# aiortc/aioquic

Hardware: AMD Instinct MI355X
Metric: GiB/s device-resident AEAD protect+unprotect, 1200B packets, 1/2/4/8 MI355X (higher is better)
Workload: dtype u8

## Files before the change

aioquic_amd/csrc/qpp_device.h:

```cpp
#pragma once

#include <hip/hip_runtime.h>
#include <stdint.h>

#include "../../include/quic_pp.h"

namespace qpp {


struct AesTables {
    uint8_t sbox[256];
    uint32_t te0[256];
};

constexpr uint8_t gf8_mul(uint8_t a, uint8_t b)
{
    uint8_t r = 0;
    for (int i = 0; i < 8; ++i) {
        if (b & 1) r ^= a;
        a = (uint8_t)((a << 1) ^ ((a & 0x80) ? 0x1b : 0));
        b >>= 1;
    }
    return r;
}
// ... 396 lines not shown
        uint32_t e[2][16];
        lds_phase_prio(true);
#pragma unroll
        for (int b = 0; b < 2; ++b) {
#pragma unroll
            for (int col = 0; col < 4; ++col) {
                e[b][4 * col + 0] = T.t0(s[b][col]);
                e[b][4 * col + 1] = T.t1(s[b][(col + 1) & 3]);
                e[b][4 * col + 2] = T.t2r(s[b][(col + 2) & 3]);
                e[b][4 * col + 3] = T.t3r(s[b][(col + 3) & 3]);
            }
        }
        __builtin_amdgcn_sched_barrier(0);
        lds_phase_prio(false);
#pragma unroll
        for (int b = 0; b < 2; ++b) {
#pragma unroll
            for (int col = 0; col < 4; ++col)
                s[b][col] = xor3(e[b][4 * col], e[b][4 * col + 1],
                                 rotl(xor3(e[b][4 * col + 2], e[b][4 * col + 3], k[col]), 16));
        }
    }
    const uint32_t *k = rk + 4 * NR;
    uint32_t f[2][16];
    lds_phase_prio(true);
#pragma unroll
    for (int b = 0; b < 2; ++b) {
#pragma unroll
        for (int col = 0; col < 4; ++col) {
            f[b][4 * col + 0] = T.fr0(s[b][col]);
            f[b][4 * col + 1] = T.fr1(s[b][(col + 1) & 3]);
            f[b][4 * col + 2] = T.fr2(s[b][(col + 2) & 3]);
            f[b][4 * col + 3] = T.fr3(s[b][(col + 3) & 3]);
        }
    }
    __builtin_amdgcn_sched_barrier(0);
    lds_phase_prio(false);
    uint32_t o[2][4];
#pragma unroll
    for (int b = 0; b < 2; ++b) {
#pragma unroll
        for (int col = 0; col < 4; ++col)
            o[b][col] = fin_col(f[b][4 * col], f[b][4 * col + 1], f[b][4 * col + 2], f[b][4 * col + 3], k[col]);
    }
    o0 = u32x4{o[0][0], o[0][1], o[0][2], o[0][3]};
    o1 = u32x4{o[1][0], o[1][1], o[1][2], o[1][3]};
}


__device__ __forceinline__ u32x4 ghash_mul(u32x4 x, const uint8_t *lds, uint32_t tab)
{
    u32x4 acc = {0, 0, 0, 0};
    uint32_t xw[4] = {x.x, x.y, x.z, x.w};
#pragma unroll
    for (int d = 0; d < 4; ++d) {
        uint32_t hi = xw[d] & 0xF0F0F0F0u;
        uint32_t lo = (xw[d] << 4) & 0xF0F0F0F0u;
#pragma unroll
        for (int b = 0; b < 4; ++b) {
            const int wlo = 2 * (4 * d + b), whi = wlo + 1;
            const uint32_t sel = 0x0c0c0c00u | (uint32_t)b;
            uint32_t alo = __builtin_amdgcn_perm(0u, lo, sel);
            uint32_t ahi = __builtin_amdgcn_perm(0u, hi, sel);
            u32x4 e0 = *(const u32x4 *)(lds + tab + wlo * 256 + alo);
            u32x4 e1 = *(const u32x4 *)(lds + tab + whi * 256 + ahi);
            acc = xor3(acc, e0, e1);
        }
    }
    return acc;
}

template <int W0, int W1>
struct Gh5Grp {
    u32x2 lo[W1 - W0], hi[W1 - W0];
    __device__ __forceinline__ void issue(const uint32_t (&xw)[4], const uint8_t *base, uint32_t tsel)
    {
#pragma unroll
        for (int i = 0; i < W1 - W0; ++i) {
            const int w = W0 + i, sb = 5 * w, d = sb >> 5, off = sb & 31;
            uint32_t e;
            if (off <= 27) asm("v_bfe_u32 %0, %1, %2, 5" : "=v"(e) : "v"(xw[d]), "i"(off));
            else if (d < 3) e = __builtin_amdgcn_alignbit(xw[d + 1], xw[d], off) & 31u;
            else e = xw[3] >> off;
            const uint32_t a = (e << 3) | tsel;
            lo[i] = *(const u32x2 *)(base + w * 256 + a);
            hi[i] = *(const u32x2 *)(base + kGh5Hi + w * 256 + a);
        }
    }
    __device__ __forceinline__ void consume(u32x4 &acc) const
    {
        constexpr int n = W1 - W0;
#pragma unroll
        for (int i = 0; i + 1 < n; i += 2) {
            acc.x = xor3(acc.x, lo[i].x, lo[i + 1].x);
            acc.y = xor3(acc.y, lo[i].y, lo[i + 1].y);
            acc.z = xor3(acc.z, hi[i].x, hi[i + 1].x);
            acc.w = xor3(acc.w, hi[i].y, hi[i + 1].y);
        }
        if constexpr (n & 1) {
            acc.x ^= lo[n - 1].x;
            acc.y ^= lo[n - 1].y;
            acc.z ^= hi[n - 1].x;
            acc.w ^= hi[n - 1].y;
        }
    }
};

__device__ __forceinline__ u32x4 ghash_mul_lds5(u32x4 x, const uint8_t *base, uint32_t tsel)
{
    const uint32_t xw[4] = {x.x, x.y, x.z, x.w};
// ... 84 lines not shown
```

aioquic_amd/csrc/qpp_engine.hip:

```cpp
#include <hip/hip_runtime.h>

#include "qpp_chacha.h"
#include "qpp_gf128.h"
#include "qpp_device.h"
#include "qpp_hkdf.h"
#include "qpp_internal.h"

namespace qpp {

__constant__ AesTables c_aes = kAesTables;

constexpr int kSetupWG = 256;
constexpr int kScratch = 112;
constexpr int kScrEj0 = 48, kScrPark = 64, kScrHdr = 96;
constexpr uint32_t kNoSlot = 0xffffffffu;
constexpr uint32_t kFlagReject = 0x8000u;
constexpr int kChachaWpe = 4;

constexpr int kChRegion = 64 * 16 + 16;
constexpr int kChStage = 4 * kChRegion;

#ifndef QPP_CH_POLY4
#define QPP_CH_POLY4 1
#endif
// ... 336 lines not shown
#define QPP_PROBE_AT(i) probe_mark(i)
#define QPP_PROBE_COUNT()                                                                     \
    do {                                                                                      \
        const uint32_t w_ = blockIdx.x * (blockDim.x / 64) + (threadIdx.x >> 6);              \
        if (w_ < kProbeWaves && __lane_id() == __ffsll((long long)__ballot(1)) - 1)           \
            atomicAdd(&g_probe[(size_t)w_ * kProbeSlots + kProbeItems], 1ull);                \
    } while (0)
#else
#define QPP_PROBE_COUNT() ((void)0)
#define QPP_PROBE_AT(i) ((void)0)
#endif

__device__ __forceinline__ void park(const Pkt &P, uint8_t *scr, bool mask = true)
{
    if (mask) *(u32x4 *)(scr + kScrPark) = P.mask;
    *(u32x4 *)(scr + kScrPark + 16) =
        u32x4{(uint32_t)P.pn, (uint32_t)(P.pn >> 32),
              P.fbm | (uint32_t)P.pn_off << 8 | (uint32_t)P.pn_len << 24 | (uint32_t)P.hp << 28,
              (uint32_t)P.hlen | (uint32_t)P.clen << 16};
}
__device__ __forceinline__ Pkt unpark(const uint8_t *scr, const uint8_t *src, uint8_t *dst, bool mask = true)
{
    Pkt P;
    const u32x4 w = *(const u32x4 *)(scr + kScrPark + 16);
    P.src = src;
    P.dst = dst;
    P.hlen = (int)(w.w & 0xffff);
    P.clen = (int)(w.w >> 16);
    P.mask = mask ? *(const u32x4 *)(scr + kScrPark) : zero4();
    P.pn = (uint64_t)w.y << 32 | w.x;
    P.fbm = w.z & 0xff;
    P.pn_off = (int)((w.z >> 8) & 0xffff);
    P.pn_len = (int)((w.z >> 24) & 0xf);
    P.hp = (w.z >> 28) & 1;
    P.status = QPP_S_OK;
    P.nonce = u32x4{0, 0, 0, 0};
    return P;
}

__device__ __forceinline__ uint32_t lds_ld(const uint32_t *p)
{
    return __hip_atomic_load(p, __ATOMIC_RELAXED, __HIP_MEMORY_SCOPE_WORKGROUP);
}
__device__ __forceinline__ void lds_st(uint32_t *p, uint32_t v)
{
    __hip_atomic_store(p, v, __ATOMIC_RELAXED, __HIP_MEMORY_SCOPE_WORKGROUP);
}

struct GhashTabs {
    const uint8_t *lds;
    const uint8_t *gtab;
    const uint32_t *wslot;
    const uint32_t *went;
    __device__ __forceinline__ uint32_t t4() const
    {
        return __builtin_amdgcn_readfirstlane(lds_ld(went)) * (uint32_t)kGhLdsEntry;
    }
    __device__ __forceinline__ const uint8_t *global(uint32_t pw) const
    {
        const uint32_t s = __builtin_amdgcn_readfirstlane(lds_ld(wslot));
        return gtab + (size_t)s * kGhashTabBytes + pw * (uint32_t)kGhashPowBytes;
    }
};

template <int BPL>
__device__ __forceinline__ int gcm_pad(int n_g)
{
    constexpr int QS = 4 * BPL;
    return QS * ((n_g + QS - 1) / QS) - n_g;
}

template <int BPL>
__device__ __forceinline__ bool gcm_fast_hp(int hlen, int clen)
{
    if constexpr (BPL != 2) {
        return false;
    } else {
        const int n_a = (hlen + 15) >> 4, n_c = (clen + 15) >> 4, za = n_a > 0 ? 1 : 0;
        return gcm_pad<BPL>(za + n_c + 1) + za <= 6 && clen >= 19;
    }
}

__device__ __forceinline__ void buf_st_part(__amdgpu_buffer_rsrc_t r, uint32_t off, u32x4 v, int n)
{
    const int nd = n >> 2, rb = n & 3;
    if (nd > 0) __builtin_amdgcn_raw_buffer_store_b32(v.x, r, (int)off, 0, 0);
    if (nd > 1) __builtin_amdgcn_raw_buffer_store_b32(v.y, r, (int)off + 4, 0, 0);
    if (nd > 2) __builtin_amdgcn_raw_buffer_store_b32(v.z, r, (int)off + 8, 0, 0);
    if (rb) {
        uint32_t t = nd == 0 ? v.x : nd == 1 ? v.y : nd == 2 ? v.z : v.w;
        const int o = (int)off + 4 * nd;
        if (rb & 2) {
            __builtin_amdgcn_raw_buffer_store_b16((unsigned short)t, r, o, 0, 0);
            t >>= 16;
        }
        if (rb & 1) __builtin_amdgcn_raw_buffer_store_b8((unsigned char)t, r, o + (rb & 2), 0, 0);
    }
}

__device__ __forceinline__ void write_header_v(const Pkt &P, int sub, bool masked, int rlen, u32x4 h0,
                                               bool have_h0)
{
    const int n_a = (P.hlen + 15) >> 4;
    for (int q = sub; q < n_a; q += 4) {
        const int nb = min(16, P.hlen - 16 * q);
        u32x4 h = (q == 0 && have_h0) ? h0 : ld_win(P.src + 16 * q, nb, P.src, P.src + rlen);
        if (masked) h ^= hp_pattern(16 * q, P.mask, P.fbm, P.pn_off, P.pn_len);
        st_part(P.dst + 16 * q, h, nb);
    }
}

template <int NR, bool ENC, int BPL, int SUITE, bool PRIO>
__device__ __forceinline__ u32x4 gcm_packet(const Pkt &P, const KeySlot *ks, const u32x4 h0,
                                            const uint32_t *rk, int sub, const GhashTabs &G,
                                            const uint8_t *te, const Bufs &B, uint32_t ioff, uint32_t ooff,
                                            u32x4 &got_tag, uint32_t pbase = 0u)
{
    const LdsTe T{te, (lane_fresh() & 31) * 4};
    const int hlen = P.hlen, clen = P.clen;
    const int n_a = (hlen + 15) >> 4, n_c = (clen + 15) >> 4, za = n_a > 0 ? 1 : 0;
    const int n_g = za + n_c + 1, pad = gcm_pad<BPL>(n_g), S = (n_g + pad) / (4 * BPL);
    const int rlen = hlen + clen + (ENC ? 0 : QPP_TAG_LEN);
    const bool tiny = rlen < 16;
    const uint32_t t4 = G.t4();
    const u32x4 tiny_in = tiny ? ld_part(P.src, rlen) : zero4();
    const int q = pad + za;
    const uint32_t cin = ioff + (uint32_t)hlen, cout = ooff + (uint32_t)hlen;
    auto ct_load = [&](int i) -> uint32_t {
        if (i < 0 || 16 * i >= clen) return kOob;
        return cin + (uint32_t)(ENC ? min(16 * i, clen - 16) : 16 * i);
    };
    u32x4 nxt0 = {0, 0, 0, 0}, nxt1 = {0, 0, 0, 0};
    if constexpr (BPL == 2) {
        nxt0 = __builtin_amdgcn_raw_buffer_load_b128(B.in, (int)ct_load(sub - q), 0, 0);
        nxt1 = __builtin_amdgcn_raw_buffer_load_b128(B.in, (int)ct_load(sub - q + 4), 0, 0);
    }

    u32x4 z = {0, 0, 0, 0};
    for (int g = 0; g < n_a; ++g) {
        u32x4 a;
        if (tiny) {
            a = tiny_in;
        } else if (g == 0) {
            a = h0;
        } else {
            const int ld = min(16 * g, rlen - 16);
            a = shr_bytes(__builtin_amdgcn_raw_buffer_load_b128(B.in, (int)(ioff + ld), 0, 0),
                          16 * g - ld);
        }
        a = keep_bytes(a, min(16, hlen - 16 * g));
        if (!ENC && P.hp) a ^= hp_pattern(16 * g, P.mask, P.fbm, P.pn_off, P.pn_len);
        if (g > 0) z = ghash_mul_global(z, G.global(0));
        z ^= a;
    }
    if (!ENC || !P.hp) write_header_v(P, sub, !ENC && P.hp, rlen, tiny ? tiny_in : h0, true);
    const bool fast_hp = ENC && P.hp && gcm_fast_hp<BPL>(hlen, clen);
    u32x4 acc = (BPL == 1 && za && sub == pad) ? z : u32x4{0, 0, 0, 0};
    const CtrCache cc = ctr_cache(P.nonce, rk, T);
    const uint32_t lens_h = bswap((uint32_t)hlen * 8u);

    auto close = [&](u32x4 ksl) {
        const uint32_t lf = lane_fresh();
        acc = ghash_mul_global(acc, G.global(3u - (lf & 3)));
        if ((lf & 3) == 3) acc ^= ksl;
    };
    auto blk_out = [&](int i, u32x4 ksb, u32x4 raw) -> u32x4 {
        const bool is_ct = i >= 0 && 16 * i < clen;
        u32x4 x = {0, 0, 0, 0}, out = {0, 0, 0, 0};
        uint32_t soff = kOob;
        if (is_ct) {
            const int nb = clen - 16 * i;
            if (__builtin_expect(nb >= 16, 1)) {
                out = raw ^ ksb;
                x = ENC ? out : raw;
                soff = cout + 16u * (uint32_t)i;
            } else {
                const u32x4 cur = ENC ? shr_bytes(raw, 16 - nb) : raw;
                out = cur ^ ksb;
                x = keep_bytes(ENC ? out : cur, nb);
                buf_st_part(B.out, cout + 16u * (uint32_t)i, out, nb);
            }
        } else if (i >= 0 && 16 * i < clen + 16) {
            x = u32x4{0u, lens_h, 0u, bswap((uint32_t)clen * 8u)};
        }
        __builtin_amdgcn_raw_buffer_store_b128(out, B.out, (int)soff, 0, 0);
        return x;
    };
    auto step = [&](int i, bool last, auto first_c, u32x4 raw) {
        (void)first_c;
        const LdsTe Tl{te, (lane_fresh() & 31) * 4};
        const bool is_ct = i >= 0 && 16 * i < clen;
        const u32x4 ksb = aes_ctr<NR>(cc, is_ct ? (uint32_t)(i + 2) : 1u, rk, Tl);
        acc ^= blk_out(i, ksb, raw);
        __builtin_amdgcn_sched_barrier(0);
        if (!last) acc = ghash_mul_h4(acc, G.lds, t4);
        else close(ksb);
    };
    auto step2 = [&](int i, bool last, u32x4 raw0, u32x4 raw1, auto first_c) {
        constexpr bool first = decltype(first_c)::value;
        const LdsTe Tl{te, (lane_fresh() & 31) * 4};
        const uint32_t cb0 = (i >= 0 && 16 * i < clen) ? (uint32_t)(i + 2) : 1u;
        const uint32_t cb1 = (i + 4 >= 0 && 16 * (i + 4) < clen) ? (uint32_t)(i + 6) : 1u;
        u32x4 ks0, ks1;
        if (first && pad >= 4) {
            ks0 = zero4();
            ks1 = aes_ctr<NR>(cc, cb1, rk, Tl);
        } else {
            aes_ctr2<NR>(cc, cb0, cb1, rk, Tl, ks0, ks1);
        }
        u32x4 x0 = blk_out(i, ks0, raw0);
        u32x4 x1 = blk_out(i + 4, ks1, raw1);
        if constexpr (first) {
            if constexpr (ENC) {
                if (fast_hp) {
                    u32x4 c0 = (i == 0) ? x0 : (i + 4 == 0) ? x1 : zero4();
                    u32x4 c1 = (i == 1) ? x0 : (i + 4 == 1) ? x1 : zero4();
// ... 432 lines not shown
        uint8_t *dst = P.dst;
        P = unpark(scr, src, dst, !ENC);
    }
    const int L = chunks & 3;
    const int nb = chunks > 0 ? n_c - 4 * (chunks - 1) : 1;
    const int role = (sub - L - 1) & 3;
    auto power = [&](int e) -> P130 {
        P130 x;
#pragma unroll
        for (int l = 0; l < 5; ++l) x.v[l] = pw[5 * e + l];
        return x;
    };
    const u32x4 lens = u32x4{(uint32_t)P.hlen, 0u, (uint32_t)P.clen, 0u};
    const P130 lb = p130_block(lens);
    P130 a = acc;
#pragma unroll
    for (int l = 0; l < 5; ++l) a.v[l] += role == 3 ? lb.v[l] : 0u;
    const P130 m = p130_mul(a, power(role == 0 ? kPw8 : role == 1 ? kPw1 + 3 : role == 2 ? kPwOne : kPw1));
    P130 u = m, v = p130_zero();
#pragma unroll
    for (int l = 0; l < 5; ++l) {
        u.v[l] = role == 3 ? 0u : m.v[l];
        v.v[l] = role == 3 ? m.v[l] : 0u;
    }
    const P130 sum = p130_add(p130_mul(p130_quad_sum(u), power(kPw1 + nb)), p130_quad_sum(v));
    const u32x4 sw = *(const u32x4 *)(scr + kScrEj0);
    const u32x4 tag = p130_finish(sum, sw.x, sw.y, sw.z, sw.w);
    if (ENC) {
        if (sub == 0) st16(pout + P.clen, tag);
        if (P.hp) protect_finish_hp<QPP_CHACHA20_POLY1305>(P, ks, sub, scr, tag, ConstTe{}, h0);
    } else {
        const u32x4 got = ld16(pin + P.clen);
        const u32x4 diff = got ^ tag;
        if ((diff.x | diff.y | diff.z | diff.w) != 0) {
            P.status = QPP_S_DECRYPT;
            wipe_payload(P, sub, [&](int i) { return ((i >> 2) + 1) & 3; });
        }
    }
    QPP_PROBE_AT(7);
}

template <bool ENC>
__device__ __forceinline__ void write_result(qpp_result *res, uint32_t p, int sub, const Pkt &P)
{
    if (sub != 0) return;
    const uint32_t out_len =
        P.status == QPP_S_OK ? (uint32_t)(P.hlen + P.clen + (ENC ? QPP_TAG_LEN : 0)) : 0u;
    res[p] = qpp_result{P.pn, (uint16_t)P.status, (uint16_t)P.hlen, out_len};
}



constexpr int kTabEntries = 4;
template <int WG>
constexpr int gcm_tab_entries() { return WG == 512 ? 1 : kTabEntries; }
static_assert(kGhLdsEntry % 1024 == 0, "LDS-DMA pieces of 1 KiB");

__device__ uint32_t g_qpp_watchdog;

__device__ uint32_t g_qpp_spin_tab = 1u << 22;
__device__ uint32_t g_qpp_spin_lone = 1u << 18;
__device__ uint32_t g_qpp_pair_delay = 0u;

template <int WG, int NE = gcm_tab_entries<WG>()>
struct __attribute__((aligned(16))) GcmSmem {
    uint8_t h4[NE][kGhLdsEntry];
    uint8_t te[kTeBytes];
    uint32_t eslot[NE];
    uint32_t eref[NE];
    uint32_t eready[NE];
    uint32_t eused[NE];

    uint32_t lock, tick, next;
    uint32_t exited;
    uint32_t wslot[WG / 64];
    uint32_t went[WG / 64];
};

template <int WG>
__device__ uint32_t tab_acquire(GcmSmem<WG> &sm, const uint8_t *gtab, uint32_t cur)
{
    const uint32_t spin = __builtin_nontemporal_load(&g_qpp_spin_tab);
    typedef const __attribute__((address_space(1))) void *gptr_t;
    typedef __attribute__((address_space(3))) void *lptr_t;
    uint32_t e = kNoSlot, load = 0;
#pragma unroll 1
    for (uint32_t it = 0; it < spin; ++it) {
        uint32_t got = kNoSlot, ld = 0;
        if (lane_fresh() == 0) {
            while (atomicCAS(&sm.lock, 0u, 1u) != 0u) __builtin_amdgcn_s_sleep(1);
            int hit = -1, vic = -1;
            uint32_t best = 0xffffffffu;
#pragma unroll
            for (int i = 0; i < gcm_tab_entries<WG>(); ++i) {
                const uint32_t s = lds_ld(&sm.eslot[i]);
                const uint32_t r = lds_ld(&sm.eref[i]);
                const uint32_t u = lds_ld(&sm.eused[i]);
                if (s == cur) hit = i;
                else if (r == 0u && u < best) {
                    best = u;
                    vic = i;
                }
            }
            if (hit < 0 && vic >= 0) {
                hit = vic;
                ld = 1;
                lds_st(&sm.eslot[vic], cur);
                lds_st(&sm.eready[vic], 0u);
            }
            if (hit >= 0) {
                got = (uint32_t)hit;
                atomicAdd(&sm.eref[hit], 1u);
                const uint32_t t = lds_ld(&sm.tick) + 1u;
                lds_st(&sm.tick, t);
                lds_st(&sm.eused[hit], t);
            }
            asm volatile("s_waitcnt lgkmcnt(0)" ::: "memory");
            atomicExch(&sm.lock, 0u);
        }
        got = __builtin_amdgcn_readfirstlane(got);
        if (got != kNoSlot) {
            e = got;
            load = __builtin_amdgcn_readfirstlane(ld);
            break;
        }
        __builtin_amdgcn_s_sleep(8);
    }
    if (e == kNoSlot) return e;
    if (load) {
        const uint8_t *src = gtab + (size_t)cur * kGhashTabBytes + kGh5Off;
        const uint32_t l = lane_fresh();
#pragma unroll
        for (int c = 0; c < kGhLdsEntry / 1024; ++c)
            __builtin_amdgcn_global_load_lds((gptr_t)(src + c * 1024 + l * 16), (lptr_t)(sm.h4[e] + c * 1024),
                                             16, 0, 0);
        asm volatile("s_waitcnt vmcnt(0)" ::: "memory");
        if (lane_fresh() == 0) lds_st(&sm.eready[e], 1u);
    } else {
        bool ready = false;
#pragma unroll 1
        for (uint32_t it = 0; it < spin; ++it) {
            if (__builtin_amdgcn_readfirstlane(lds_ld(&sm.eready[e]))) {
                ready = true;
                break;
            }
            __builtin_amdgcn_s_sleep(2);
        }
        if (!ready) {
            if (lane_fresh() == 0) atomicSub(&sm.eref[e], 1u);
            return kNoSlot;
        }
    }
    return e;
}

template <int WG>
__device__ __forceinline__ void tab_release(GcmSmem<WG> &sm, uint32_t e)
{
    if (lane_fresh() == 0) atomicSub(&sm.eref[e], 1u);
}

#ifdef QPP_STUDY_SYNTH
__device__ __forceinline__ qpp_desc study_desc(const qpp_desc *, uint32_t p)
{
    return qpp_desc{1200ull * p, 1200ull * p, 1173u, 11, 0, (uint64_t)p, 0u, p};
}
#define QPP_DESC(i) study_desc(desc, (i))
#else
#define QPP_DESC(i) desc[i]
#endif

#ifndef QPP_POOL_DIV
#define QPP_POOL_DIV 12
#endif
constexpr uint32_t kPoolDiv = QPP_POOL_DIV;
#ifndef QPP_POOL512
#define QPP_POOL512 0
#endif
#ifndef QPP_COMBO_PRIO
#define QPP_COMBO_PRIO 0
#endif
#ifndef QPP_SHARE_PRIO
#define QPP_SHARE_PRIO 0
#endif
#ifndef QPP_PRIO512
#define QPP_PRIO512 1
#endif

template <int SUITE, bool ENC, int WG, int BPL>
__global__ __launch_bounds__(WG) __attribute__((amdgpu_waves_per_eu(4))) void k_gcm(const KeySlot *__restrict__ slots,
                                              const uint8_t *__restrict__ gtab, uint32_t cap,
                                              const qpp_desc *__restrict__ desc, uint32_t n,
                                              const uint8_t *gin, uint8_t *gout,
                                              qpp_result *__restrict__ res,
                                              const uint32_t *__restrict__ items,
                                              const uint32_t *__restrict__ irange,
                                              uint32_t *__restrict__ pool)
{
    constexpr int kNR = SUITE == QPP_AES_256_GCM ? 14 : 10;
    const uint32_t wv = __builtin_amdgcn_readfirstlane(threadIdx.x >> 6);
    QPP_PROBE_AT(kProbeStart);
    const bool planned = irange != nullptr;
    uint32_t ib = 0, ie = (n + 15u) / 16u;
    if (planned) {
        ib = irange[2 * SUITE];
        ie = irange[2 * SUITE + 1];
    }
    const uint32_t total = ie > ib ? ie - ib : 0u;
    const uint32_t pool_n = pool ? total / kPoolDiv : 0u, stat = total - pool_n;
    const uint32_t per = (stat + gridDim.x - 1) / gridDim.x;
    const uint32_t sb = ib + min(stat, per * blockIdx.x), se = ib + min(stat, per * (blockIdx.x + 1));
    if (!pool && sb >= se) return;
    __shared__ GcmSmem<WG> sm;
    auto tid_now = [&]() -> uint32_t { return (wv << 6) | lane_fresh(); };
    load_te<WG>(sm.te);
    if (threadIdx.x < gcm_tab_entries<WG>()) {
        sm.eslot[threadIdx.x] = kNoSlot;
        sm.eref[threadIdx.x] = 0u;
        sm.eready[threadIdx.x] = 0u;
        sm.eused[threadIdx.x] = 0u;
    }
    if (threadIdx.x == 0) {
        sm.lock = 0u;
        sm.tick = 0u;
        sm.next = sb;
        sm.exited = 0u;
    }
    if (threadIdx.x < WG / 64) sm.wslot[threadIdx.x] = kNoSlot;
    __syncthreads();
    QPP_PROBE_AT(0);

#pragma unroll 1
    for (;;) {
        uint32_t j = 0;
        if (lane_fresh() == 0) j = atomicAdd(&sm.next, 1u);
        j = __builtin_amdgcn_readfirstlane(j);
        if (j >= se) {
            if (!pool) break;
            uint32_t q = 0;
            if (lane_fresh() == 0) q = atomicAdd(&pool[0], 1u);
            q = __builtin_amdgcn_readfirstlane(q);
            if (q >= pool_n) break;
            j = ib + stat + q;
        }
#if QPP_COMBO_PRIO
        uint32_t pbase = 0u;
        if constexpr (WG == 512) pbase = (j < se && 2u * (se - j) > se - sb) ? 2u : 0u;
#endif
#if QPP_SHARE_PRIO
        if constexpr (WG == 512) {
            const uint32_t tot = se - sb, rem = j < se ? se - j : 0u;
            const uint32_t pr = tot ? min(3u, (4u * rem) / (tot + 1u)) : 0u;
            if (pr >= 3) __builtin_amdgcn_s_setprio(3);
            else if (pr == 2) __builtin_amdgcn_s_setprio(2);
            else if (pr == 1) __builtin_amdgcn_s_setprio(1);
            else __builtin_amdgcn_s_setprio(0);
        }
#endif
        QPP_PROBE_AT(1);
        QPP_PROBE_COUNT();
        uint32_t wb, we;
        if (planned) {
            wb = __builtin_amdgcn_readfirstlane(items[j]);
            we = __builtin_amdgcn_readfirstlane(items[j + 1]);
        } else {
            wb = 16u * j;
            we = min(n, wb + 16u);
        }
        auto pkt_of = [&](uint32_t t) -> uint32_t { return wb + ((t & 63) >> 2); };
        auto slot_of = [&](const qpp_desc &d, uint32_t p) -> uint32_t {
            return (p < we && d.slot < cap) ? d.slot : kNoSlot;
        };
        uint64_t bi, bo;
        {
            const uint32_t t = tid_now(), p = pkt_of(t);
            uint64_t in0 = ~0ull, out0 = ~0ull;
            if (p < we) {
                const qpp_desc d = QPP_DESC(p);
                in0 = d.in_off;
                out0 = d.out_off;
                if (d.slot >= cap && (t & 3) == 0) res[planned ? d.rsv : p] = qpp_result{d.pn, QPP_S_NO_KEY, 0, 0};
            }
            bi = wave_min_u64(in0);
            bo = wave_min_u64(out0);
        }

        auto run_slot = [&](uint32_t cur) {
            const KeySlot *ks = slots + cur;
            const uint32_t t1 = tid_now(), p1 = pkt_of(t1);
            const qpp_desc d = p1 < we ? QPP_DESC(p1) : qpp_desc{0, 0, 0, 0, 0, 0, kNoSlot, 0};
            if (slot_of(d, p1) != cur) return;
#ifdef QPP_STUDY_SYNTH
            const HdrPre pre = {{0x41u, 0, 0, 0}, {0, 0, 0, 0}, {0, 0, 0, 0}, 0x41u};
#else
            const HdrPre pre = prefetch_hdr<ENC>(d, gin, true);
#endif
            const LdsTe T{sm.te, (t1 & 31) * 4};
            Pkt P = pkt_begin<ENC, SUITE>(d, pre, gin, gout, ks, T);
            if (P.status == QPP_S_OK) {
                uint32_t rk[4 * (kNR + 1)];
#pragma unroll
                for (int i = 0; i < 4 * (kNR + 1); ++i)
                    rk[i] = __builtin_amdgcn_readfirstlane((i >= 12 && i < 4 * kNR) ? ks->rkr[i] : ks->rk[i]);
                const uint64_t ioff = d.in_off - bi, ooff = d.out_off - bo;
                if (item_span_ok<ENC>(P, ioff, ooff)) {
                    const Bufs B{
                        __builtin_amdgcn_make_buffer_rsrc((void *)(gin + bi), 0, (int)kBufBytes, 0x00020000),
                        __builtin_amdgcn_make_buffer_rsrc((void *)(gout + bo), 0, (int)kBufBytes, 0x00020000)};
                    const GhashTabs G{&sm.h4[0][0], gtab, &sm.wslot[wv], &sm.went[wv]};
                    QPP_PROBE_AT(3);
                    const uint64_t pn = P.pn;
                    const int hlen = P.hlen;
                    u32x4 got_tag;
                    const u32x4 tag = gcm_packet<kNR, ENC, BPL, SUITE, WG == 512 && QPP_PRIO512>(P, ks, pre.h0, rk, t1 & 3, G, sm.te, B,
                                                                       (uint32_t)ioff, (uint32_t)ooff, got_tag
#if QPP_COMBO_PRIO
                                                                       , pbase
#endif
                                                                       );
                    QPP_PROBE_AT(6);
                    const uint32_t t2 = tid_now(), p2 = pkt_of(t2);
                    const qpp_desc d2 = QPP_DESC(p2);
                    Pkt Q;
                    Q.src = gin + d2.in_off;
                    Q.dst = gout + d2.out_off;
                    Q.hp = !(d2.flags & QPP_F_NO_HP);
                    Q.status = QPP_S_OK;
                    Q.hlen = ENC ? (int)d2.hdr_len : hlen;
                    Q.clen = ENC ? (int)d2.len : (int)d2.len - hlen - QPP_TAG_LEN;
                    Q.pn = ENC ? d2.pn : pn;
                    Q.pn_off = Q.pn_len = 0;
                    Q.fbm = 0;
                    Q.mask = zero4();
                    Q.nonce = zero4();
                    const LdsTe T2{sm.te, (t2 & 31) * 4};
                    const KeySlot *ks2 =
                        slots + __builtin_amdgcn_readfirstlane(lds_ld(&sm.wslot[wv]));
                    gcm_finish<ENC, SUITE, BPL>(Q, ks2, t2 & 3, T2, tag, got_tag);
                    P = Q;
                } else {
                    P.status = QPP_S_LENGTH;
                }
            }
            const uint32_t t3 = tid_now(), p3 = pkt_of(t3);
            write_result<ENC>(res, planned ? QPP_DESC(p3).rsv : p3, t3 & 3, P);
            QPP_PROBE_AT(7);
        };

        uint32_t last = kNoSlot;
#pragma unroll 1
        for (int guard = 0; guard < 17; ++guard) {
            const uint32_t t = tid_now(), p = pkt_of(t);
            const uint32_t s = p < we ? slot_of(QPP_DESC(p), p) : kNoSlot;
            const uint32_t cur = wave_min_u32((last == kNoSlot || s > last) ? s : kNoSlot);
            if (cur == kNoSlot) break;
            last = cur;
            const bool final_slot = __builtin_amdgcn_ballot_w64(s != kNoSlot && s > cur) == 0;
            const uint32_t held = __builtin_amdgcn_readfirstlane(lds_ld(&sm.wslot[wv]));
            const uint32_t suite =
                cur == held ? (uint32_t)SUITE : __builtin_amdgcn_readfirstlane(slots[cur].suite);
            uint32_t fail = 0u;
            if (suite > QPP_CHACHA20_POLY1305) {
                fail = QPP_S_NO_KEY;
            } else if (suite != SUITE) {
                continue;
            } else if (cur != held) {
                QPP_PROBE_AT(1);
                if (held != kNoSlot) {
                    tab_release<WG>(sm, __builtin_amdgcn_readfirstlane(lds_ld(&sm.went[wv])));
                    if (lane_fresh() == 0) lds_st(&sm.wslot[wv], kNoSlot);
                }
                const uint32_t e = tab_acquire<WG>(sm, gtab, cur);
                if (e == kNoSlot) {
                    if (lane_fresh() == 0) atomicAdd(&g_qpp_watchdog, 1u);
                    fail = QPP_S_INTERNAL;
                } else if (lane_fresh() == 0) {
                    lds_st(&sm.wslot[wv], cur);
                    lds_st(&sm.went[wv], e);
                }
            }
            if (fail) {
                if (s == cur && (t & 3) == 0) {
                    const qpp_desc d = QPP_DESC(p);
                    res[planned ? d.rsv : p] = qpp_result{d.pn, (uint16_t)fail, 0, 0};
                }
                continue;
            }
            QPP_PROBE_AT(2);
            run_slot(cur);
            QPP_PROBE_AT(8);
            if (final_slot) break;
        }
    }
    if (__builtin_amdgcn_readfirstlane(lds_ld(&sm.wslot[wv])) != kNoSlot)
        tab_release<WG>(sm, __builtin_amdgcn_readfirstlane(lds_ld(&sm.went[wv])));
    if (pool && lane_fresh() == 0 && atomicAdd(&sm.exited, 1u) == (uint32_t)(WG / 64 - 1) &&
        atomicAdd(&pool[1], 1u) == gridDim.x - 1) {
        atomicExch(&pool[0], 0u);
        atomicExch(&pool[1], 0u);
    }
    QPP_PROBE_AT(9);
}

struct WaveSpan {
    uint32_t b, e;
    bool empty_wg;
};
template <int WG, int SUITE>
__device__ __forceinline__ WaveSpan wave_span(uint32_t n, const uint32_t *items, const uint32_t *irange,
                                              uint32_t wv, uint32_t blk)
{
    constexpr uint32_t kWaves = WG / 64;
    WaveSpan w{0u, 0u, false};
    if (irange) {
        const uint32_t ib = irange[2 * SUITE], ie = irange[2 * SUITE + 1];
        const uint32_t j0 = ib + blk * kWaves;
        w.empty_wg = j0 >= ie;
        const uint32_t j = j0 + wv;
        if (j < ie) {
            w.b = __builtin_amdgcn_readfirstlane(items[j]);
            w.e = __builtin_amdgcn_readfirstlane(items[j + 1]);
        }
    } else {
        const uint32_t b0 = blk * (kWaves * 16u);
        w.empty_wg = b0 >= n;
        w.b = b0 + wv * 16u;
        w.e = w.b < n ? min(n, w.b + 16u) : w.b;
    }
    return w;
}

template <bool ENC, int WG, bool PRIO>
__device__ __forceinline__ void chacha_wave(const WaveSpan &W, ChachaSmem<WG> &sm, const KeySlot *__restrict__ slots,
                                            uint32_t cap, const qpp_desc *__restrict__ desc, const uint8_t *gin,
                                            uint8_t *gout, qpp_result *__restrict__ res,
                                            const uint32_t *__restrict__ irange)
{
    constexpr int SUITE = QPP_CHACHA20_POLY1305;
#ifdef QPP_CH_STAGGER
    {
        const uint32_t slot = __builtin_amdgcn_s_getreg(4 | (0 << 6) | (3 << 11));
        for (uint32_t i = 0; i < slot * QPP_CH_STAGGER; ++i) __builtin_amdgcn_s_sleep(1);
    }
#endif
    QPP_PROBE_AT(kProbeStart);
    if constexpr (PRIO) __builtin_amdgcn_s_setprio(3);
    const uint32_t lim = W.e, planned = irange != nullptr;
    auto p_now = [&]() -> uint32_t { return W.b + (lane_fresh() >> 2); };
// ... 715 lines not shown

}


#include <stdlib.h>
#include <string.h>

#include <algorithm>
#include <immintrin.h>
#include <pthread.h>

#include <atomic>
#include <chrono>
#include <condition_variable>
#include <deque>
#include <mutex>
#include <thread>
#include <vector>

using namespace qpp;

constexpr int kPoolSlots = 32;
constexpr uint32_t kPoolStride = 32;
struct PoolRing {
    std::mutex mu;
    uint32_t *d = nullptr;
    hipEvent_t ev[kPoolSlots] = {};
    uint8_t state[kPoolSlots] = {};
    int next = 0;
};

struct qpp_keytab {
    uint32_t cap;
    int device;
    KeySlot *d_slots;
    uint8_t *d_gtab;
    qpp_key_material *d_km;
    uint32_t km_cap;
    uint8_t *h_suite;
    uint32_t n_suite[3];
    PoolRing *pool;
};

static bool pool_choice()
{
    static const bool b = [] {
        const char *v = getenv("QPP_GCM_POOL");
        return !(v && v[0] == '0');
    }();
    return b;
}

static std::atomic<uint64_t> g_pool_fallbacks{0};

static int pool_acquire(const qpp_keytab *kt)
{
    PoolRing *r = kt->pool;
    if (!r || !pool_choice()) return -1;
    std::lock_guard<std::mutex> l(r->mu);
    for (int i = 0; i < kPoolSlots; ++i) {
        const int sl = (r->next + i) % kPoolSlots;
        if (r->state[sl] == 1) continue;
        if (r->state[sl] == 2) {
            const hipError_t q = hipEventQuery(r->ev[sl]);
            if (q != hipSuccess) {
                (void)hipGetLastError();
                continue;
            }
        } else if (!r->ev[sl] && hipEventCreateWithFlags(&r->ev[sl], hipEventDisableTiming) != hipSuccess) {
            (void)hipGetLastError();
            r->ev[sl] = nullptr;
            continue;
        }
        r->state[sl] = 1;
        r->next = (sl + 1) % kPoolSlots;
        return sl;
    }
    g_pool_fallbacks.fetch_add(1, std::memory_order_relaxed);
    return -1;
}

static void pool_release(const qpp_keytab *kt, int sl, hipStream_t s)
{
    if (sl < 0) return;
    PoolRing *r = kt->pool;
    std::lock_guard<std::mutex> l(r->mu);
    if (hipEventRecord(r->ev[sl], s) != hipSuccess) {
        (void)hipGetLastError();
        r->state[sl] = 1;
        return;
    }
    r->state[sl] = 2;
}

static void keytab_note(qpp_keytab *kt, uint32_t slot, uint32_t suite)
{
    const uint8_t old = kt->h_suite[slot];
    if (old <= QPP_CHACHA20_POLY1305) --kt->n_suite[old];
    kt->h_suite[slot] = (uint8_t)suite;
    if (suite <= QPP_CHACHA20_POLY1305) ++kt->n_suite[suite];
}

static uint32_t keytab_suite_mask(const qpp_keytab *kt)
{
    uint32_t m = 0;
    for (int s = 0; s < 3; ++s)
        if (kt->n_suite[s]) m |= 1u << s;
    return m;
}

constexpr size_t kPipeChunkBytes = (size_t)32 << 20;
constexpr int kPipeRegular = 32, kPipeTaper = 2;
constexpr int kPipeMaxChunks = kPipeRegular + 2 * kPipeTaper;
constexpr int kMultiMaxDevices = 16;

struct qpp_session {
    hipStream_t stream;
    hipStream_t s_in, s_out;
    hipEvent_t ev_in[kPipeMaxChunks], ev_k[kPipeMaxChunks], ev_out[kPipeMaxChunks];
    int device;
    size_t max_bytes;
    uint32_t max_packets;
    uint8_t *h_in, *h_out, *h_misc;
    uint8_t *hd_in, *hd_out, *hd_misc;
    uint8_t *d_in, *d_out, *d_misc;
    size_t misc_bytes;
    qpp_plan *plan;
    bool trace;
    hipEvent_t tev[6][kPipeMaxChunks];
    qpp_trace last;
};

constexpr uint32_t kSessionPlanMin = 128;

#define HIPCHK(x)                          \
    do {                                   \
        if ((x) != hipSuccess) {           \
            (void)hipGetLastError();       \
            return QPP_E_HIP;              \
        }                                  \
    } while (0)

extern "C" {

int qpp_abi_version(void) { return QPP_ABI_VERSION; }

uint64_t qpp_pool_fallbacks(void) { return g_pool_fallbacks.load(std::memory_order_relaxed); }

uint32_t qpp_watchdog_count(void)
{
    uint32_t v = 0;
    if (hipMemcpyFromSymbol(&v, HIP_SYMBOL(g_qpp_watchdog), sizeof v, 0, hipMemcpyDeviceToHost) != hipSuccess) {
        (void)hipGetLastError();
        return 0;
    }
    return v;
}

const char *qpp_strerror(int rc)
{
    switch (rc) {
    case QPP_OK: return "ok";
    case QPP_E_ARG: return "invalid argument";
    case QPP_E_HIP: return "HIP runtime error";
    case QPP_E_NODEV: return "no gfx950 device";
    case QPP_E_NOMEM: return "out of memory";
    default: return "unknown error";
    }
}

int qpp_device_check(void)
{
    int dev = 0, count = 0;
    if (hipGetDeviceCount(&count) != hipSuccess || count < 1) {
        (void)hipGetLastError();
        return QPP_E_NODEV;
    }
    HIPCHK(hipGetDevice(&dev));
    hipDeviceProp_t prop;
    HIPCHK(hipGetDeviceProperties(&prop, dev));
    return strncmp(prop.gcnArchName, "gfx950", 6) == 0 ? QPP_OK : QPP_E_NODEV;
}

int qpp_keytab_create(uint32_t capacity, qpp_keytab **out)
{
    if (!out || capacity == 0 || capacity > (1u << 24)) return QPP_E_ARG;
    *out = NULL;
    int rc = qpp_device_check();
    if (rc != QPP_OK) return rc;
    qpp_keytab *kt = (qpp_keytab *)calloc(1, sizeof(qpp_keytab));
    if (!kt) return QPP_E_NOMEM;
    kt->cap = capacity;
    (void)hipGetDevice(&kt->device);
    kt->h_suite = (uint8_t *)malloc(capacity);
    if (!kt->h_suite) {
        free(kt);
        return QPP_E_NOMEM;
    }
    memset(kt->h_suite, 0xff, capacity);
    kt->pool = new (std::nothrow) PoolRing();
// ... 203 lines not shown
    (void)hipGetDevice(&dev);
    if (dev < 0 || dev >= 64) dev = 0;
    if (!cus[dev]) {
        int c = 0;
        if (hipDeviceGetAttribute(&c, hipDeviceAttributeMultiprocessorCount, dev) != hipSuccess || c < 1) {
            (void)hipGetLastError();
            c = 256;
        }
        cus[dev] = c;
    }
    return (uint32_t)cus[dev];
}

static uint32_t gcm_grid(uint32_t items, uint32_t waves_per_wg)
{
    const uint32_t need = (items + waves_per_wg - 1) / waves_per_wg;
    const uint32_t cap = cu_count() * (waves_per_wg == 8 ? 2u : 1u);
    return need < cap ? (need ? need : 1u) : cap;
}

#ifndef QPP_TWO_WG_ITEMS
#define QPP_TWO_WG_ITEMS 16u
#endif
static bool gcm_two_wg(const qpp_keytab *kt, uint32_t suite, uint32_t items)
{
    return kt->n_suite[suite] == 1 && items <= cu_count() * (uint32_t)QPP_TWO_WG_ITEMS;
}

static bool chacha_prio(uint32_t waves)
{
    static const int m = [] {
        const char *v = getenv("QPP_CHACHA_PRIO");
        return v ? atoi(v) : 1;
    }();
    return m == 2 || (m == 1 && waves <= cu_count() * 4u * kChachaWpe);
}

static int launch_packets(bool enc, const qpp_keytab *kt, const qpp_desc *d_desc, uint32_t n,
                          const uint8_t *d_in, uint8_t *d_out, qpp_result *d_res, void *stream,
                          const qpp_plan *plan = nullptr, const LoneStage *stage = nullptr)
{
    if (!kt || (n && (!d_desc || !d_in || !d_out || !d_res))) return QPP_E_ARG;
    if (n == 0) return QPP_OK;
    hipStream_t s = (hipStream_t)stream;
    if (int rc = apply_spin_env(s)) return rc;
    uint32_t mask = keytab_suite_mask(kt);
    if (!mask && !plan) mask = 1u;
    const uint32_t *d_items = plan ? plan->d_items : nullptr, *d_irange = plan ? plan->d_irange : nullptr;
    const uint32_t waves = plan ? qpp_internal_plan_max_items(n, kt->cap) : (n + 15) / 16;
    const int bpl_gcm = gcm_bpl_choice();
    const bool lone = !plan && lone_choice();
    const dim3 lgrid((n + kLoneWG / 64 - 1) / (kLoneWG / 64)), lblock(kLoneWG);
    const LoneStage lst = stage ? *stage : LoneStage{nullptr, nullptr, 0u};
#define QPP_LAUNCH_GCM_W(SUITE, BPLV, WGV)                                                     \
    do {                                                                                       \
        const dim3 grid(gcm_grid(waves, WGV / 64)), block(WGV);                                 \
        const int psl = (WGV == 1024 || QPP_POOL512) && kt->n_suite[SUITE] == 1 ? pool_acquire(kt) : -1; \
        uint32_t *pl = psl >= 0 ? kt->pool->d + (size_t)psl * kPoolStride : nullptr;          \
        if (enc)                                                                               \
            hipLaunchKernelGGL((k_gcm<SUITE, true, WGV, BPLV>), grid, block, 0, s,             \
                               kt->d_slots, kt->d_gtab, kt->cap, d_desc, n, d_in, d_out, d_res, \
                               d_items, d_irange, pl);                                         \
        else                                                                                   \
            hipLaunchKernelGGL((k_gcm<SUITE, false, WGV, BPLV>), grid, block, 0, s,            \
                               kt->d_slots, kt->d_gtab, kt->cap, d_desc, n, d_in, d_out, d_res, \
                               d_items, d_irange, pl);                                         \
        pool_release(kt, psl, s);                                                              \
    } while (0)
#define QPP_LAUNCH_GCM_B(SUITE, BPLV)                                                          \
    do {                                                                                       \
        if (BPLV == 2 && gcm_two_wg(kt, SUITE, waves)) QPP_LAUNCH_GCM_W(SUITE, BPLV, 512);       \
        else QPP_LAUNCH_GCM_W(SUITE, BPLV, kGcmWG);                                             \
    } while (0)
#define QPP_LAUNCH_GCM(SUITE)                                                                  \
    if (mask & (1u << SUITE)) {                                                                \
        if (lone && n <= lone_max(SUITE)) {                                                    \
            if (enc)                                                                           \
                hipLaunchKernelGGL((k_lone_gcm<SUITE, true>), lgrid, lblock, 0, s, kt->d_slots, \
                                   kt->d_gtab, kt->cap, d_desc, n, d_in, d_out, d_res, lst);   \
            else                                                                               \
                hipLaunchKernelGGL((k_lone_gcm<SUITE, false>), lgrid, lblock, 0, s, kt->d_slots, \
                                   kt->d_gtab, kt->cap, d_desc, n, d_in, d_out, d_res, lst);   \
        } else if (bpl_gcm == 1) {                                                             \
            QPP_LAUNCH_GCM_B(SUITE, 1);                                                         \
        } else {                                                                               \
            QPP_LAUNCH_GCM_B(SUITE, 2);                                                         \
        }                                                                                      \
        HIPCHK(hipGetLastError());                                                             \
    }
    QPP_LAUNCH_GCM(QPP_AES_128_GCM)
    QPP_LAUNCH_GCM(QPP_AES_256_GCM)
    if ((mask & (1u << QPP_CHACHA20_POLY1305)) && lone && n <= lone_max(QPP_CHACHA20_POLY1305)) {
        if (enc)
            hipLaunchKernelGGL((k_lone_chacha<true>), lgrid, lblock, 0, s, kt->d_slots, kt->cap, d_desc, n, d_in,
                               d_out, d_res, lst);
        else
            hipLaunchKernelGGL((k_lone_chacha<false>), lgrid, lblock, 0, s, kt->d_slots, kt->cap, d_desc, n, d_in,
                               d_out, d_res, lst);
        HIPCHK(hipGetLastError());
    } else if (mask & (1u << QPP_CHACHA20_POLY1305)) {
        uint32_t cgrid = (waves + kChachaWG / 64 - 1) / (kChachaWG / 64);
        if (QPP_CH_PERSIST > 0) {
            const uint32_t resident = cu_count() * (uint32_t)(4 * kChachaWpe / (kChachaWG / 64)) * (uint32_t)QPP_CH_PERSIST;
            cgrid = cgrid < resident ? cgrid : resident;
        }
        const dim3 grid(cgrid ? cgrid : 1u), block(kChachaWG);
        if (chacha_prio(waves)) {
            if (enc)
                hipLaunchKernelGGL((k_chacha<true, kChachaWG, true>), grid, block, 0, s, kt->d_slots, kt->cap,
                                   d_desc, n, d_in, d_out, d_res, d_items, d_irange);
            else
                hipLaunchKernelGGL((k_chacha<false, kChachaWG, true>), grid, block, 0, s, kt->d_slots, kt->cap,
                                   d_desc, n, d_in, d_out, d_res, d_items, d_irange);
        } else if (enc) {
            hipLaunchKernelGGL((k_chacha<true, kChachaWG, false>), grid, block, 0, s, kt->d_slots, kt->cap,
                               d_desc, n, d_in, d_out, d_res, d_items, d_irange);
        } else {
            hipLaunchKernelGGL((k_chacha<false, kChachaWG, false>), grid, block, 0, s, kt->d_slots, kt->cap,
                               d_desc, n, d_in, d_out, d_res, d_items, d_irange);
        }
        HIPCHK(hipGetLastError());
    }
#undef QPP_LAUNCH_GCM
#undef QPP_LAUNCH_GCM_B
#undef QPP_LAUNCH_GCM_W
// ... 921 lines not shown
```

include/quic_pp.h:

```cpp
#ifndef QUIC_PP_H
#define QUIC_PP_H

#include <stddef.h>
#include <stdint.h>

#ifdef __cplusplus
extern "C" {
#endif

#define QPP_ABI_VERSION 3

#define QPP_AES_128_GCM 0
#define QPP_AES_256_GCM 1
#define QPP_CHACHA20_POLY1305 2

#define QPP_PACKET_MAX 1500
#define QPP_TAG_LEN 16
#define QPP_MAX_HDR 1500
#define QPP_ITEM_SPAN_MAX 0xffffff00u

#define QPP_OK 0
#define QPP_E_ARG (-1)
#define QPP_E_HIP (-2)
#define QPP_E_NODEV (-3)
// ... 7 lines not shown
#define QPP_S_INTERNAL 5

#define QPP_F_NO_HP 1u
#define QPP_F_RFC_PN 2u

typedef struct qpp_desc {
    uint64_t in_off;
    uint64_t out_off;
    uint32_t len;
    uint16_t hdr_len;
    uint16_t flags;
    uint64_t pn;
    uint32_t slot;
    uint32_t rsv;
} qpp_desc;

typedef struct qpp_result {
    uint64_t pn;
    uint16_t status;
    uint16_t hdr_len;
    uint32_t out_len;
} qpp_result;

typedef struct qpp_key_material {
    uint32_t slot;
    uint8_t suite;
    uint8_t key_phase;
    uint8_t rsv[2];
    uint8_t iv[12];
    uint8_t key[32];
    uint8_t hp[32];
} qpp_key_material;

#define QPP_DERIVE_V2 1u

typedef struct qpp_secret {
    uint32_t slot;
    uint8_t suite;
    uint8_t key_phase;
    uint8_t flags;
    uint8_t secret_len;
    uint32_t updates;
    uint32_t rsv;
    uint8_t secret[64];
} qpp_secret;

typedef struct qpp_keytab qpp_keytab;
typedef struct qpp_session qpp_session;

int qpp_abi_version(void);
const char *qpp_source_hash(void);
uint32_t qpp_watchdog_count(void);
uint64_t qpp_pool_fallbacks(void);
const char *qpp_strerror(int rc);
int qpp_device_check(void);

int qpp_keytab_create(uint32_t capacity, qpp_keytab **out);
void qpp_keytab_destroy(qpp_keytab *kt);
uint32_t qpp_keytab_capacity(const qpp_keytab *kt);
int qpp_keytab_set(qpp_keytab *kt, const qpp_key_material *km, uint32_t n, void *stream);
int qpp_keytab_clear(qpp_keytab *kt, const uint32_t *slots, uint32_t n, void *stream);
int qpp_keytab_derive(qpp_keytab *kt, const qpp_secret *sec, uint32_t n,
                      qpp_key_material *km_out, void *stream);

int qpp_protect(const qpp_keytab *kt, const qpp_desc *d_desc, uint32_t n, const uint8_t *d_in,
                uint8_t *d_out, qpp_result *d_res, void *stream);
int qpp_unprotect(const qpp_keytab *kt, const qpp_desc *d_desc, uint32_t n,
                  const uint8_t *d_in, uint8_t *d_out, qpp_result *d_res, void *stream);

typedef struct qpp_plan qpp_plan;
int qpp_plan_create(uint32_t max_packets, qpp_plan **out);
void qpp_plan_destroy(qpp_plan *p);
int qpp_plan_build(qpp_plan *p, const qpp_keytab *kt, const qpp_desc *d_desc, uint32_t n,
                   void *stream);
int qpp_protect_planned(const qpp_keytab *kt, const qpp_plan *p, const qpp_desc *d_desc,
                        uint32_t n, const uint8_t *d_in, uint8_t *d_out, qpp_result *d_res,
                        void *stream);
int qpp_unprotect_planned(const qpp_keytab *kt, const qpp_plan *p, const qpp_desc *d_desc,
                          uint32_t n, const uint8_t *d_in, uint8_t *d_out, qpp_result *d_res,
                          void *stream);

int qpp_hp_mask(const qpp_keytab *kt, const uint32_t *d_slots, const uint8_t *d_samples,
                uint32_t n, uint8_t *d_masks, void *stream);

int qpp_session_create(size_t max_bytes, uint32_t max_packets, qpp_session **out);
void qpp_session_destroy(qpp_session *s);
void *qpp_session_stream(qpp_session *s);
int qpp_session_protect(qpp_session *s, const qpp_keytab *kt, const qpp_desc *desc, uint32_t n,
                        const uint8_t *in, size_t in_len, uint8_t *out, size_t out_len,
                        qpp_result *res);
int qpp_session_unprotect(qpp_session *s, const qpp_keytab *kt, const qpp_desc *desc,
                          uint32_t n, const uint8_t *in, size_t in_len, uint8_t *out,
                          size_t out_len, qpp_result *res);
int qpp_session_hp_mask(qpp_session *s, const qpp_keytab *kt, const uint32_t *slots,
                        const uint8_t *samples, uint32_t n, uint8_t *masks);
int qpp_session_stage(qpp_session *s, size_t bytes, uint32_t n, uint8_t **h_in, uint8_t **h_out);
int qpp_session_set_keys(qpp_session *s, qpp_keytab *kt, const qpp_key_material *km,
                         uint32_t n);

typedef struct qpp_trace {
    uint32_t pipelined;
    uint32_t chunks;
    double total_ms;
    double submit_ms;
    double copy_in_ms;
    double copy_out_ms;
// ... 26 lines not shown
```

Before: 448.0.

## Cache GHASH close-power tables in LDS for single-key 1024-thread GCM launches

Adds a kernel variant (CLDS) for the 1024-thread GCM path with a single key suite. It shrinks the H^4 LDS table cache to one entry and reuses the freed space to DMA the full GHASH power tables into LDS. The multiplies for the GHASH close and the header use LDS lookups instead of global-table lookups when the resident slot matches the current key. The cost is less H^4 table caching and an extra per-workgroup table load. Separately, the outer loop of ghash_mul is no longer unrolled, which lowers code size and register pressure at some loop overhead.

```diff
diff --git a/aioquic_amd/csrc/qpp_device.h b/aioquic_amd/csrc/qpp_device.h
--- a/aioquic_amd/csrc/qpp_device.h
+++ b/aioquic_amd/csrc/qpp_device.h
@@ -472,10 +472,11 @@
 {
     u32x4 acc = {0, 0, 0, 0};
     uint32_t xw[4] = {x.x, x.y, x.z, x.w};
-#pragma unroll
+#pragma unroll 1
     for (int d = 0; d < 4; ++d) {
-        uint32_t hi = xw[d] & 0xF0F0F0F0u;
-        uint32_t lo = (xw[d] << 4) & 0xF0F0F0F0u;
+        const uint32_t w = d == 0 ? xw[0] : d == 1 ? xw[1] : d == 2 ? xw[2] : xw[3];
+        uint32_t hi = w & 0xF0F0F0F0u;
+        uint32_t lo = (w << 4) & 0xF0F0F0F0u;
 #pragma unroll
         for (int b = 0; b < 4; ++b) {
             const int wlo = 2 * (4 * d + b), whi = wlo + 1;
diff --git a/aioquic_amd/csrc/qpp_engine.hip b/aioquic_amd/csrc/qpp_engine.hip
--- a/aioquic_amd/csrc/qpp_engine.hip
+++ b/aioquic_amd/csrc/qpp_engine.hip
@@ -412,6 +412,8 @@
     const uint8_t *gtab;
     const uint32_t *wslot;
     const uint32_t *went;
+    const uint8_t *ctab;
+    const uint32_t *cslot;
     __device__ __forceinline__ uint32_t t4() const
     {
         return __builtin_amdgcn_readfirstlane(lds_ld(went)) * (uint32_t)kGhLdsEntry;
@@ -420,6 +422,10 @@
     {
         const uint32_t s = __builtin_amdgcn_readfirstlane(lds_ld(wslot));
         return gtab + (size_t)s * kGhashTabBytes + pw * (uint32_t)kGhashPowBytes;
+    }
+    __device__ __forceinline__ bool close_resident() const
+    {
+        return __builtin_amdgcn_readfirstlane(lds_ld(cslot)) == __builtin_amdgcn_readfirstlane(lds_ld(wslot));
     }
 };
 
@@ -470,7 +476,7 @@
     }
 }
 
-template <int NR, bool ENC, int BPL, int SUITE, bool PRIO>
+template <int NR, bool ENC, int BPL, int SUITE, bool PRIO, bool CLDS = false>
 __device__ __forceinline__ u32x4 gcm_packet(const Pkt &P, const KeySlot *ks, const u32x4 h0,
                                             const uint32_t *rk, int sub, const GhashTabs &G,
                                             const uint8_t *te, const Bufs &B, uint32_t ioff, uint32_t ooff,
@@ -496,6 +502,12 @@
         nxt1 = __builtin_amdgcn_raw_buffer_load_b128(B.in, (int)ct_load(sub - q + 4), 0, 0);
     }
 
+    auto mul_pow = [&](u32x4 x, uint32_t pw) -> u32x4 {
+        if constexpr (CLDS) {
+            if (G.close_resident()) return ghash_mul(x, G.ctab, pw * (uint32_t)kGhashPowBytes);
+        }
+        return ghash_mul_global(x, G.global(pw));
+    };
     u32x4 z = {0, 0, 0, 0};
     for (int g = 0; g < n_a; ++g) {
         u32x4 a;
@@ -510,7 +522,7 @@
         }
         a = keep_bytes(a, min(16, hlen - 16 * g));
         if (!ENC && P.hp) a ^= hp_pattern(16 * g, P.mask, P.fbm, P.pn_off, P.pn_len);
-        if (g > 0) z = ghash_mul_global(z, G.global(0));
+        if (g > 0) z = mul_pow(z, 0u);
         z ^= a;
     }
     if (!ENC || !P.hp) write_header_v(P, sub, !ENC && P.hp, rlen, tiny ? tiny_in : h0, true);
@@ -521,7 +533,7 @@
 
     auto close = [&](u32x4 ksl) {
         const uint32_t lf = lane_fresh();
-        acc = ghash_mul_global(acc, G.global(3u - (lf & 3)));
+        acc = mul_pow(acc, 3u - (lf & 3));
         if ((lf & 3) == 3) acc ^= ksl;
     };
     auto blk_out = [&](int i, u32x4 ksb, u32x4 raw) -> u32x4 {
@@ -1060,9 +1072,12 @@
 
 
 constexpr int kTabEntries = 4;
-template <int WG>
-constexpr int gcm_tab_entries() { return WG == 512 ? 1 : kTabEntries; }
+template <int WG, bool CLDS = false>
+constexpr int gcm_tab_entries() { return (WG == 512 || CLDS) ? 1 : kTabEntries; }
 static_assert(kGhLdsEntry % 1024 == 0, "LDS-DMA pieces of 1 KiB");
+constexpr int kCloseTabBytes = kGhashPowers * kGhashPowBytes;
+static_assert(kCloseTabBytes % 1024 == 0 && kCloseTabBytes <= (kTabEntries - 1) * kGhLdsEntry,
+              "the close tables fit the space of the H^4 entries they replace");
 
 __device__ uint32_t g_qpp_watchdog;
 
@@ -1070,9 +1085,13 @@
 __device__ uint32_t g_qpp_spin_lone = 1u << 18;
 __device__ uint32_t g_qpp_pair_delay = 0u;
 
-template <int WG, int NE = gcm_tab_entries<WG>()>
+template <int WG, bool CLDS = false, int NE = gcm_tab_entries<WG, CLDS>()>
 struct __attribute__((aligned(16))) GcmSmem {
+    static constexpr int kEntries = NE;
+    static constexpr bool kClose = CLDS;
     uint8_t h4[NE][kGhLdsEntry];
+    uint8_t ctab[CLDS ? kCloseTabBytes : 0];
+    uint32_t cslot[CLDS ? 4 : 0];
     uint8_t te[kTeBytes];
     uint32_t eslot[NE];
     uint32_t eref[NE];
@@ -1085,8 +1104,8 @@
     uint32_t went[WG / 64];
 };
 
-template <int WG>
-__device__ uint32_t tab_acquire(GcmSmem<WG> &sm, const uint8_t *gtab, uint32_t cur)
+template <class SM>
+__device__ uint32_t tab_acquire(SM &sm, const uint8_t *gtab, uint32_t cur)
 {
     const uint32_t spin = __builtin_nontemporal_load(&g_qpp_spin_tab);
     typedef const __attribute__((address_space(1))) void *gptr_t;
@@ -1100,7 +1119,7 @@
             int hit = -1, vic = -1;
             uint32_t best = 0xffffffffu;
 #pragma unroll
-            for (int i = 0; i < gcm_tab_entries<WG>(); ++i) {
+            for (int i = 0; i < SM::kEntries; ++i) {
                 const uint32_t s = lds_ld(&sm.eslot[i]);
                 const uint32_t r = lds_ld(&sm.eref[i]);
                 const uint32_t u = lds_ld(&sm.eused[i]);
@@ -1115,6 +1134,12 @@
                 ld = 1;
                 lds_st(&sm.eslot[vic], cur);
                 lds_st(&sm.eready[vic], 0u);
+                if constexpr (SM::kClose) {
+                    if (lds_ld(&sm.cslot[0]) == kNoSlot) {
+                        lds_st(&sm.cslot[0], cur);
+                        ld = 3;
+                    }
+                }
             }
             if (hit >= 0) {
                 got = (uint32_t)hit;
@@ -1142,6 +1167,15 @@
         for (int c = 0; c < kGhLdsEntry / 1024; ++c)
             __builtin_amdgcn_global_load_lds((gptr_t)(src + c * 1024 + l * 16), (lptr_t)(sm.h4[e] + c * 1024),
                                              16, 0, 0);
+        if constexpr (SM::kClose) {
+            if (load & 2u) {
+                const uint8_t *src4 = gtab + (size_t)cur * kGhashTabBytes;
+#pragma unroll 4
+                for (int c = 0; c < kCloseTabBytes / 1024; ++c)
+                    __builtin_amdgcn_global_load_lds((gptr_t)(src4 + c * 1024 + l * 16),
+                                                     (lptr_t)(sm.ctab + c * 1024), 16, 0, 0);
+            }
+        }
         asm volatile("s_waitcnt vmcnt(0)" ::: "memory");
         if (lane_fresh() == 0) lds_st(&sm.eready[e], 1u);
     } else {
@@ -1162,8 +1196,8 @@
     return e;
 }
 
-template <int WG>
-__device__ __forceinline__ void tab_release(GcmSmem<WG> &sm, uint32_t e)
+template <class SM>
+__device__ __forceinline__ void tab_release(SM &sm, uint32_t e)
 {
     if (lane_fresh() == 0) atomicSub(&sm.eref[e], 1u);
 }
@@ -1195,7 +1229,7 @@
 #define QPP_PRIO512 1
 #endif
 
-template <int SUITE, bool ENC, int WG, int BPL>
+template <int SUITE, bool ENC, int WG, int BPL, bool CLDS = false>
 __global__ __launch_bounds__(WG) __attribute__((amdgpu_waves_per_eu(4))) void k_gcm(const KeySlot *__restrict__ slots,
                                               const uint8_t *__restrict__ gtab, uint32_t cap,
                                               const qpp_desc *__restrict__ desc, uint32_t n,
@@ -1219,10 +1253,11 @@
     const uint32_t per = (stat + gridDim.x - 1) / gridDim.x;
     const uint32_t sb = ib + min(stat, per * blockIdx.x), se = ib + min(stat, per * (blockIdx.x + 1));
     if (!pool && sb >= se) return;
-    __shared__ GcmSmem<WG> sm;
+    static_assert(!CLDS || WG == 1024, "the 512-thread shape has no LDS to spare for the close tables");
+    __shared__ GcmSmem<WG, CLDS> sm;
     auto tid_now = [&]() -> uint32_t { return (wv << 6) | lane_fresh(); };
     load_te<WG>(sm.te);
-    if (threadIdx.x < gcm_tab_entries<WG>()) {
+    if (threadIdx.x < gcm_tab_entries<WG, CLDS>()) {
         sm.eslot[threadIdx.x] = kNoSlot;
         sm.eref[threadIdx.x] = 0u;
         sm.eready[threadIdx.x] = 0u;
@@ -1233,6 +1268,7 @@
         sm.tick = 0u;
         sm.next = sb;
         sm.exited = 0u;
+        if constexpr (CLDS) sm.cslot[0] = kNoSlot;
     }
     if (threadIdx.x < WG / 64) sm.wslot[threadIdx.x] = kNoSlot;
     __syncthreads();
@@ -1315,12 +1351,12 @@
                     const Bufs B{
                         __builtin_amdgcn_make_buffer_rsrc((void *)(gin + bi), 0, (int)kBufBytes, 0x00020000),
                         __builtin_amdgcn_make_buffer_rsrc((void *)(gout + bo), 0, (int)kBufBytes, 0x00020000)};
-                    const GhashTabs G{&sm.h4[0][0], gtab, &sm.wslot[wv], &sm.went[wv]};
+                    const GhashTabs G{&sm.h4[0][0], gtab, &sm.wslot[wv], &sm.went[wv], sm.ctab, sm.cslot};
                     QPP_PROBE_AT(3);
                     const uint64_t pn = P.pn;
                     const int hlen = P.hlen;
                     u32x4 got_tag;
-                    const u32x4 tag = gcm_packet<kNR, ENC, BPL, SUITE, WG == 512 && QPP_PRIO512>(P, ks, pre.h0, rk, t1 & 3, G, sm.te, B,
+                    const u32x4 tag = gcm_packet<kNR, ENC, BPL, SUITE, WG == 512 && QPP_PRIO512, CLDS>(P, ks, pre.h0, rk, t1 & 3, G, sm.te, B,
                                                                        (uint32_t)ioff, (uint32_t)ooff, got_tag
 #if QPP_COMBO_PRIO
                                                                        , pbase
@@ -1375,10 +1411,10 @@
             } else if (cur != held) {
                 QPP_PROBE_AT(1);
                 if (held != kNoSlot) {
-                    tab_release<WG>(sm, __builtin_amdgcn_readfirstlane(lds_ld(&sm.went[wv])));
+                    tab_release(sm, __builtin_amdgcn_readfirstlane(lds_ld(&sm.went[wv])));
                     if (lane_fresh() == 0) lds_st(&sm.wslot[wv], kNoSlot);
                 }
-                const uint32_t e = tab_acquire<WG>(sm, gtab, cur);
+                const uint32_t e = tab_acquire(sm, gtab, cur);
                 if (e == kNoSlot) {
                     if (lane_fresh() == 0) atomicAdd(&g_qpp_watchdog, 1u);
                     fail = QPP_S_INTERNAL;
@@ -1401,7 +1437,7 @@
         }
     }
     if (__builtin_amdgcn_readfirstlane(lds_ld(&sm.wslot[wv])) != kNoSlot)
-        tab_release<WG>(sm, __builtin_amdgcn_readfirstlane(lds_ld(&sm.went[wv])));
+        tab_release(sm, __builtin_amdgcn_readfirstlane(lds_ld(&sm.went[wv])));
     if (pool && lane_fresh() == 0 && atomicAdd(&sm.exited, 1u) == (uint32_t)(WG / 64 - 1) &&
         atomicAdd(&pool[1], 1u) == gridDim.x - 1) {
         atomicExch(&pool[0], 0u);
@@ -2223,6 +2259,7 @@
 }
 
 static std::atomic<uint64_t> g_pool_fallbacks{0};
+static std::atomic<uint64_t> g_close_lds_launches{0};
 
 static int pool_acquire(const qpp_keytab *kt)
 {
@@ -2317,6 +2354,7 @@
 int qpp_abi_version(void) { return QPP_ABI_VERSION; }
 
 uint64_t qpp_pool_fallbacks(void) { return g_pool_fallbacks.load(std::memory_order_relaxed); }
+uint64_t qpp_close_lds_launches(void) { return g_close_lds_launches.load(std::memory_order_relaxed); }
 
 uint32_t qpp_watchdog_count(void)
 {
@@ -2626,25 +2664,27 @@
     const bool lone = !plan && lone_choice();
     const dim3 lgrid((n + kLoneWG / 64 - 1) / (kLoneWG / 64)), lblock(kLoneWG);
     const LoneStage lst = stage ? *stage : LoneStage{nullptr, nullptr, 0u};
-#define QPP_LAUNCH_GCM_W(SUITE, BPLV, WGV)                                                     \
+#define QPP_LAUNCH_GCM_W(SUITE, BPLV, WGV, CLDSV)                                              \
     do {                                                                                       \
         const dim3 grid(gcm_grid(waves, WGV / 64)), block(WGV);                                 \
         const int psl = (WGV == 1024 || QPP_POOL512) && kt->n_suite[SUITE] == 1 ? pool_acquire(kt) : -1; \
         uint32_t *pl = psl >= 0 ? kt->pool->d + (size_t)psl * kPoolStride : nullptr;          \
+        if (CLDSV) g_close_lds_launches.fetch_add(1, std::memory_order_relaxed);               \
         if (enc)                                                                               \
-            hipLaunchKernelGGL((k_gcm<SUITE, true, WGV, BPLV>), grid, block, 0, s,             \
+            hipLaunchKernelGGL((k_gcm<SUITE, true, WGV, BPLV, CLDSV>), grid, block, 0, s,      \
                                kt->d_slots, kt->d_gtab, kt->cap, d_desc, n, d_in, d_out, d_res, \
                                d_items, d_irange, pl);                                         \
         else                                                                                   \
-            hipLaunchKernelGGL((k_gcm<SUITE, false, WGV, BPLV>), grid, block, 0, s,            \
+            hipLaunchKernelGGL((k_gcm<SUITE, false, WGV, BPLV, CLDSV>), grid, block, 0, s,     \
                                kt->d_slots, kt->d_gtab, kt->cap, d_desc, n, d_in, d_out, d_res, \
                                d_items, d_irange, pl);                                         \
         pool_release(kt, psl, s);                                                              \
     } while (0)
 #define QPP_LAUNCH_GCM_B(SUITE, BPLV)                                                          \
     do {                                                                                       \
-        if (BPLV == 2 && gcm_two_wg(kt, SUITE, waves)) QPP_LAUNCH_GCM_W(SUITE, BPLV, 512);       \
-        else QPP_LAUNCH_GCM_W(SUITE, BPLV, kGcmWG);                                             \
+        if (BPLV == 2 && gcm_two_wg(kt, SUITE, waves)) QPP_LAUNCH_GCM_W(SUITE, BPLV, 512, false); \
+        else if (!plan && kt->n_suite[SUITE] == 1) QPP_LAUNCH_GCM_W(SUITE, BPLV, kGcmWG, true);  \
+        else QPP_LAUNCH_GCM_W(SUITE, BPLV, kGcmWG, false);                                      \
     } while (0)
 #define QPP_LAUNCH_GCM(SUITE)                                                                  \
     if (mask & (1u << SUITE)) {                                                                \
diff --git a/include/quic_pp.h b/include/quic_pp.h
--- a/include/quic_pp.h
+++ b/include/quic_pp.h
@@ -83,6 +83,7 @@
 const char *qpp_source_hash(void);
 uint32_t qpp_watchdog_count(void);
 uint64_t qpp_pool_fallbacks(void);
+uint64_t qpp_close_lds_launches(void);
 const char *qpp_strerror(int rc);
 int qpp_device_check(void);
 
```

Result: faster. 465.2, median of 6 (+3.8%).
